# NoahVl/Explaining-In-Style-Reproducibility-Study

Hardware: AMD Instinct MI355X
Metric: StylEx G+D+enc train-step images/sec @256px (higher is better)
Workload: dtype bf16; 1 GPU; FFHQ-shaped 256x256 StylEx, batch 32/GPU, GAE=2 (noise+encoder micro-steps), GP every 4th step, ResNet-18 classifier; image_size=256, batch_per_gpu=32, start_step=0, gradient_accumulate_every=2, global_batch=32, parallelism=dp1

## Files before the change

explaining-in-style-reproducibility-study_amd/csrc/conv_gather.hip:

```cpp
#include <hip/hip_runtime.h>
#include <stdint.h>
#include <stdlib.h>

#include "conv_prims.h"
#include "stylex_internal.h"


namespace {


constexpr int GBM = 128, GBN = 128;
constexpr int RING = 4;

struct GatherParams {
    const unsigned short* x;
    const unsigned short* w;
    float* partial;
    unsigned short* y;
    int B, H, W, C, N, KH, pad, sign;
    int Hs, Ws, stride;
    int m_tiles;
    int M, stages, ksplit, stages_per_split;
};


constexpr int LROW = 128;
constexpr int LSTAGE = (GBM + GBN) * LROW;
constexpr int LPIECES = 4;

__device__ __forceinline__ void lds16(bf16x8& dst, int addr) {
    asm volatile("ds_read_b128 %0, %1" : "=v"(dst) : "v"(addr));
}

__global__ __launch_bounds__(512, 1) void conv_gather_line_kernel(GatherParams p) {
    extern __shared__ __attribute__((aligned(16))) char smem[];
    const int tid = threadIdx.x, lane = tid & 63;
    const int wave = __builtin_amdgcn_readfirstlane(tid >> 6);
    const int n_tiles = (p.N + GBN - 1) / GBN;
    const int n0 = (int)(blockIdx.x % n_tiles) * GBN;
    int mt = (int)(blockIdx.x / n_tiles);
    const bool phased = p.sign < 0 && p.stride == 2;
    int py = 0, px = 0;
    if (phased) {
        const int tpp = p.m_tiles >> 2;
        const int ph = mt / tpp;
        mt -= ph * tpp;
        py = ph >> 1;
        px = ph & 1;
    }
    const int m0 = mt * GBM;
    const int rows = phased ? p.B * p.Hs * p.Ws : p.M;
    const int cpt = p.C >> 6;
    const int ks = blockIdx.y;
    const int s_begin = ks * p.stages_per_split;
    const int s_end = min(s_begin + p.stages_per_split, phased ? (1 + py) * (1 + px) * cpt : p.stages);
    const int nst = max(s_end - s_begin, 0);
    const int T = p.KH * p.KH, K = T * p.C;

    const bool stage_w = wave >= 4;
    const int rbase = (wave & 3) * 32 + (lane >> 3);
    const int Hs = __builtin_amdgcn_readfirstlane(p.Hs), Ws = __builtin_amdgcn_readfirstlane(p.Ws);
    const int C = __builtin_amdgcn_readfirstlane(p.C), KH = __builtin_amdgcn_readfirstlane(p.KH);
    const int pad = __builtin_amdgcn_readfirstlane(p.pad), sgn = __builtin_amdgcn_readfirstlane(p.sign);
    const int strd = __builtin_amdgcn_readfirstlane(p.stride);
    const int gw = phased ? Ws : p.W;
    const int hw = phased ? Hs * Ws : p.H * p.W;
    const __amdgpu_buffer_rsrc_t rx = __builtin_amdgcn_make_buffer_rsrc(const_cast<unsigned short*>(p.x), 0, 0x7ffffff0, 0x00020000);
// ... 77 lines not shown
#pragma unroll
        for (int e = 0; e < 16; ++e) acc[j][e] = 0.f;

    for (int s = 0; s < 3 && s < nst; ++s) issue_stage(s);
    for (int s = 0; s < nst; ++s) {
        if (s + 2 < nst) asm volatile("s_waitcnt vmcnt(%0)" ::"n"(2 * LPIECES) : "memory");
        else if (s + 1 < nst) asm volatile("s_waitcnt vmcnt(%0)" ::"n"(LPIECES) : "memory");
        else asm volatile("s_waitcnt vmcnt(0)" ::: "memory");
        asm volatile("s_waitcnt lgkmcnt(0)" ::: "memory");
        __builtin_amdgcn_s_barrier();
        asm volatile("" ::: "memory");
        if (s + 3 < nst) issue_stage((s + 3) % RING);
        const int base = (s % RING) * LSTAGE;
        bf16x8 av[2], bv[2][2];
        lds16(av[0], base + a_off + (s0 << 4));
        lds16(bv[0][0], base + b_off + (s0 << 4));
        lds16(bv[0][1], base + b_off + 32 * LROW + (s0 << 4));
#pragma unroll
        for (int g = 0; g < 4; ++g) {
            if (g < 3) {
                const int so = ((2 * (g + 1)) ^ s0) << 4;
                lds16(av[(g + 1) & 1], base + a_off + so);
                lds16(bv[(g + 1) & 1][0], base + b_off + so);
                lds16(bv[(g + 1) & 1][1], base + b_off + 32 * LROW + so);
                asm volatile("s_waitcnt lgkmcnt(3)" : "+v"(av[g & 1]), "+v"(bv[g & 1][0]), "+v"(bv[g & 1][1]));
            } else {
                asm volatile("s_waitcnt lgkmcnt(0)" : "+v"(av[g & 1]), "+v"(bv[g & 1][0]), "+v"(bv[g & 1][1]));
            }
#pragma unroll
            for (int j = 0; j < 2; ++j) acc[j] = __builtin_amdgcn_mfma_f32_32x32x16_bf16(av[g & 1], bv[g & 1][j], acc[j], 0, 0, 0);
        }
    }

    float* out = p.partial + (long)ks * p.M * p.N;
#pragma unroll
    for (int j = 0; j < 2; ++j) {
        const int n = n0 + wn * 64 + j * 32 + li;
#pragma unroll
        for (int r = 0; r < 16; ++r) {
            int mm = m0 + wm * 32 + (r & 3) + 8 * (r >> 2) + 4 * lk;
            const bool ok = mm < rows && n < p.N;
            if (phased && ok) {
                const int bb = mm / hw, qq = mm - bb * hw;
                const int qh = qq / p.Ws, qw = qq - qh * p.Ws;
                mm = (bb * p.H + 2 * qh + py) * p.W + 2 * qw + px;
            }
            if (ok && p.y) p.y[(long)mm * p.N + n] = act_bf16_1(acc[j][r]);
            else if (ok) out[(long)mm * p.N + n] = acc[j][r];
        }
    }
}

}

static bool gather_applicable(const ConvKParams& p) {
    const char* env = getenv("STYLEX_CONV_GATHER");
    if (env && env[0] == '0') return false;
    if (env && env[0] == 's' && p.stride != 1) return false;
    if (!p.act_bf16 || p.a_scale || p.s2d_c) return false;
    if (p.KH != p.KW || !((p.KH == 3 && p.pad == 1) || (p.KH == 1 && p.pad == 0))) return false;
    if (p.stride == 1) {
        if (p.Hi != p.Ho || p.Wi != p.Wo || p.phase_major) return false;
    } else {
        if (p.stride != 2 || p.KH != 3) return false;
        if (p.transposed ? (p.Ho != 2 * p.Hi || p.Wo != 2 * p.Wi) : (p.Hi != 2 * p.Ho || p.Wi != 2 * p.Wo)) return false;
    }
    if ((p.transposed && p.stride == 2 ? p.Hi * p.Wi : p.Ho * p.Wo) > 64) return false;
    if (p.Ck % 64 != 0 || p.N % 8 != 0 || p.N < 64) return false;
    if ((reinterpret_cast<uintptr_t>(p.a) & 15) || (reinterpret_cast<uintptr_t>(p.w) & 15)) return false;
    return true;
}

static int gather_m_tiles(const ConvKParams& p) {
    if (p.transposed && p.stride == 2) return 4 * ((p.B * p.Hi * p.Wi + GBM - 1) / GBM);
    return (p.M + GBM - 1) / GBM;
}

static int gather_stages(const ConvKParams& p) {
    return (p.transposed && p.stride == 2 ? 4 : p.KH * p.KW) * (p.Ck / 64);
}

static void gather_plan(const ConvKParams& p, int* ksplit, int* per) {
    const int stages = gather_stages(p);
    const long tiles = (long)gather_m_tiles(p) * ((p.N + GBN - 1) / GBN);
    int ks = (int)((256 + tiles - 1) / tiles);
    if (ks > stages / 4) ks = stages / 4;
    if (ks < 1) ks = 1;
    int pp = (stages + ks - 1) / ks;
    *per = pp;
    *ksplit = (stages + pp - 1) / pp;
}

int64_t stylex_gather_workspace_bytes(const ConvKParams& p) {
    if (!gather_applicable(p)) return 0;
    int ks, per;
    gather_plan(p, &ks, &per);
    return (int64_t)ks * p.M * p.N * (int64_t)sizeof(float);
}

int stylex_launch_gather(ConvKParams& p, void* workspace, int64_t workspace_bytes, hipStream_t s) {
    if (!gather_applicable(p) || !workspace) return STYLEX_NOT_APPLICABLE;
    int ks, per;
    gather_plan(p, &ks, &per);
    if (workspace_bytes < (int64_t)ks * p.M * p.N * (int64_t)sizeof(float)) return STYLEX_NOT_APPLICABLE;
    if (reinterpret_cast<uintptr_t>(workspace) & 15) return STYLEX_NOT_APPLICABLE;
    if (stylex_dynamic_lds_once<conv_gather_line_kernel>(RING * LSTAGE) != hipSuccess) {
        (void)hipGetLastError();
        return STYLEX_NOT_APPLICABLE;
    }
    GatherParams g;
    g.x = reinterpret_cast<const unsigned short*>(p.a);
    g.w = reinterpret_cast<const unsigned short*>(p.w);
    g.partial = (float*)workspace;
    const bool direct = ks == 1 && p.flags == 0 && !p.out_scale && !p.bias;
    g.y = direct ? reinterpret_cast<unsigned short*>(p.y) : nullptr;
    g.B = p.B;
    g.H = p.Ho;
    g.W = p.Wo;
    g.C = p.Ck;
    g.N = p.N;
    g.KH = p.KH;
    g.pad = p.pad;
    g.sign = p.transposed ? -1 : 1;
    g.Hs = p.Hi;
    g.Ws = p.Wi;
    g.stride = p.stride;
    g.m_tiles = gather_m_tiles(p);
    g.M = p.M;
    g.stages = gather_stages(p);
    g.ksplit = ks;
    g.stages_per_split = per;
    const long tiles = (long)g.m_tiles * ((p.N + GBN - 1) / GBN);
    stylex_note_kernel("conv_gather_line_kernel");
    hipLaunchKernelGGL(conv_gather_line_kernel, dim3((unsigned)tiles, (unsigned)ks), dim3(512), RING * LSTAGE, s, g);
    p.ksplit = direct ? 0 : ks;
    p.kt_per_split = per;
    p.partial = (float*)workspace;
    return (int)hipGetLastError();
}
```

explaining-in-style-reproducibility-study_amd/csrc/conv_igemm.hip:

```cpp
#include <hip/hip_runtime.h>
#include <stdint.h>

#include "conv_prims.h"
#include "stylex_internal.h"


namespace {

constexpr int BK = 32;


struct RowPix {
    int b, oh, ow;
    bool valid;
};

__device__ __forceinline__ RowPix decode_row(const ConvKParams& p, int m) {
    RowPix r;
    r.valid = m < p.M;
    int mm = r.valid ? m : 0;
    if (p.phase_major) {
        int hh = p.Ho >> 1, wh = p.Wo >> 1;
        int per = p.B * hh * wh;
        int ph = mm / per;
// ... 739 lines not shown
        const unsigned mb = (unsigned)((pairs + 7) / 8);
        hipLaunchKernelGGL((wgrad_reduce_small_kernel<8, 32>), dim3(mb + extra), dim3(256), 0, s, partial, dw, N, C, T, splits,
                           (int)mb, bias_part, db, wo.scale, wo.accumulate);
    } else if (T <= 9 && splits >= 16 && pairs <= 16384) {
        const unsigned mb = (unsigned)((pairs + 31) / 32);
        hipLaunchKernelGGL((wgrad_reduce_small_kernel<32, 8>), dim3(mb + extra), dim3(256), 0, s, partial, dw, N, C, T, splits,
                           (int)mb, bias_part, db, wo.scale, wo.accumulate);
    } else {
        const unsigned mb = (unsigned)((pairs + 255) / 256);
        hipLaunchKernelGGL(wgrad_reduce_kernel, dim3(mb + extra), dim3(256), 0, s, partial, dw, N, C, T, splits, (int)mb,
                           bias_part, db, wo.scale, wo.accumulate);
    }
}

template <typename OUT>
__device__ __forceinline__ OUT cvt_out(float v);
template <>
__device__ __forceinline__ float cvt_out<float>(float v) { return v; }
template <>
__device__ __forceinline__ unsigned short cvt_out<unsigned short>(float v) { return act_bf16_1(v); }

template <typename OUT>
__global__ void pack_weight_kernel(const float* __restrict__ w, OUT* __restrict__ wf, OUT* __restrict__ wb, int N,
                                   int C, int T) {
    long total = (long)N * C * T;
    for (long i = blockIdx.x * (long)blockDim.x + threadIdx.x; i < total; i += (long)gridDim.x * blockDim.x) {
        int t = (int)(i % T);
        int c = (int)((i / T) % C);
        int n = (int)(i / ((long)T * C));
        OUT v = cvt_out<OUT>(w[i]);
        if (wf) wf[((long)n * T + t) * C + c] = v;
        if (wb) wb[((long)c * T + t) * N + n] = v;
    }
}

__device__ __forceinline__ float splitk_finish(const ConvKParams& p, float v, long o, int n, int b, int oh, int ow) {
    if (p.flags & STYLEX_EPI_OSCALE) v *= p.out_scale[(long)b * p.N + n];
    if (p.flags & STYLEX_EPI_BIAS) v += p.bias[n];
    if (p.flags & STYLEX_EPI_NOISE)
        v += ((p.flags & STYLEX_EPI_NOISE_NAT) ? p.noise[((long)b * p.noise_stride + oh) * p.noise_stride + ow]
                                               : p.noise[((long)b * p.noise_stride + ow) * p.noise_stride + oh]) * p.noise_w[n] + p.noise_b[n];
    if (p.flags & STYLEX_EPI_RESIDUAL) v = (v + act_ld1(p.residual, o, p.act_bf16)) * p.res_scale;
    if (p.flags & STYLEX_EPI_GATE) v = act_ld1(p.residual, o, p.act_bf16) > 0.f ? v : p.res_scale * v;
    if (p.flags & (STYLEX_EPI_LRELU | STYLEX_EPI_RELU)) v = v > 0.f ? v : ((p.flags & STYLEX_EPI_RELU) ? 0.f : 0.2f * v);
    return v;
}

template <bool VEC>
__global__ void splitk_epilogue_kernel(ConvKParams p) {
    const long total = (long)p.M * p.N;
    if (VEC) {
        const int tot = (int)total, N = p.N, hw = p.Ho * p.Wo;
        const bool need_pix = p.flags & (STYLEX_EPI_OSCALE | STYLEX_EPI_NOISE);
        for (int o = (blockIdx.x * blockDim.x + threadIdx.x) * 4; o < tot; o += gridDim.x * blockDim.x * 4) {
            float4 v = make_float4(0.f, 0.f, 0.f, 0.f);
            for (int s = 0; s < p.ksplit; ++s) {
                const float4 t = *reinterpret_cast<const float4*>(p.partial + (long)s * total + o);
                v.x += t.x; v.y += t.y; v.z += t.z; v.w += t.w;
            }
            const int pix = o / N, n = o - pix * N;
            int b = 0, oh = 0, ow = 0;
            if (need_pix) {
                b = pix / hw;
                const int q = pix - b * hw;
                oh = q / p.Wo;
                ow = q - oh * p.Wo;
            }
            float r[4] = {v.x, v.y, v.z, v.w};
#pragma unroll
            for (int e = 0; e < 4; ++e) r[e] = splitk_finish(p, r[e], (long)o + e, n + e, b, oh, ow);
            if (p.act_bf16) {
                uint2 h;
                h.x = act_pack2(r[0], r[1]);
                h.y = act_pack2(r[2], r[3]);
                *reinterpret_cast<uint2*>(reinterpret_cast<unsigned short*>(p.y) + o) = h;
            } else {
                *reinterpret_cast<float4*>(reinterpret_cast<float*>(p.y) + o) = make_float4(r[0], r[1], r[2], r[3]);
            }
// ... 309 lines not shown
```

explaining-in-style-reproducibility-study_amd/csrc/stylex_capi.hip:

```cpp
#include <hip/hip_runtime.h>
#include <stdint.h>
#include <stdarg.h>
#include <stdio.h>
#include <string.h>

#include <array>
#include <map>
#include <mutex>
#include <string>
#include <vector>

#include "stylex_internal.h"

namespace {

typedef std::array<int64_t, 9> LayerKey;
struct TimedLaunch {
    hipEvent_t start, stop;
    int cls;
    double flops;
    double bytes;
    LayerKey key;
    char kernel[112];
};
// ... 205 lines not shown

static void fwd_params(ConvKParams& p, const int64_t* sh) {
    fill_common(p, sh);
    p.Hi = (int)sh[1];
    p.Wi = (int)sh[2];
    p.Ck = (int)sh[3];
    p.N = (int)sh[4];
    p.Ho = (int)sh[9];
    p.Wo = (int)sh[10];
    p.M = p.B * p.Ho * p.Wo;
}

static void bwd_data_params(ConvKParams& p, const int64_t* sh) {
    fill_common(p, sh);
    p.Hi = (int)sh[9];
    p.Wi = (int)sh[10];
    p.Ck = (int)sh[4];
    p.N = (int)sh[3];
    p.Ho = (int)sh[1];
    p.Wo = (int)sh[2];
    p.M = p.B * p.Ho * p.Wo;
}

int64_t stylex_conv2d_workspace_bytes(const int64_t* sh, int which, int precision) {
    if (!conv_shape_ok(sh) || (which != 0 && which != 1)) return STYLEX_EINVAL;
    ConvKParams p;
    if (which == 0) fwd_params(p, sh);
    else {
        bwd_data_params(p, sh);
        p.transposed = 1;
    }
    p.act_bf16 = precision == STYLEX_BF16_ACT;
    return stylex_igemm_workspace_bytes(p, precision);
}

int stylex_conv_mask_supported(const int64_t* sh, int which, int flags, int precision) {
    if (!conv_shape_ok(sh) || precision != STYLEX_BF16_ACT || (which != 0 && which != 1)) return 0;
    static const uintptr_t fake = 4096;
    ConvKParams p;
    if (which == 0) {
        if (!(flags & STYLEX_EPI_MASK_OUT) || !(flags & STYLEX_EPI_LRELU)) return 0;
        fwd_params(p, sh);
        if (p.N % 8 != 0) return 0;
        p.mask = (unsigned char*)fake;
    } else {
        if (!(flags & STYLEX_EPI_GATE_MASK) || (flags & ~(STYLEX_EPI_GATE_MASK))) return 0;
        bwd_data_params(p, sh);
        if (p.KH != 3 || p.stride != 1 || p.pad != 1) return 0;
        p.flip_taps = 1;
        p.gate_mask = (const unsigned char*)fake;
    }
    p.a = (const float*)fake;
    p.w = (const void*)fake;
    p.y = (float*)fake;
    p.bias = (const float*)fake;
    p.flags = flags;
    p.act_bf16 = 1;
    p.dry = 1;
    if (which == 0 && stylex_launch_rgb(p, nullptr) == 0) return 1;
    return stylex_launch_halo(p, nullptr) == 0 ? 1 : 0;
}

int stylex_conv2d_fwd(const void* x, const void* w_fwd, void* y, const int64_t* sh, int flags,
                      const stylex_conv_epilogue* epi, int precision, void* workspace, int64_t workspace_bytes,
                      void* stream) {
    if (!x || !w_fwd || !y || !conv_shape_ok(sh)) return STYLEX_EINVAL;
// ... 263 lines not shown
```

explaining-in-style-reproducibility-study_amd/csrc/stylex_internal.h:

```cpp
#pragma once
#include <hip/hip_runtime.h>
#include <stdint.h>

#include "../../include/stylex_hip.h"
#include "act_io.h"

struct ConvKParams {
    const float* a;
    const float* a_scale;
    const void* w;
    const float* a2;
    const float* a2_scale;
    float* y;
    const float* bias;
    const float* out_scale;
    const float* noise;
    const float* noise_w;
    const float* noise_b;
    const float* residual;
    float res_scale;
    int noise_stride;
    int B, Hi, Wi, Ck, N, KH, KW, Ho, Wo, stride, pad;
    int transposed;
    int phase_major;
    int act_bf16;
    int s2d_c;
    int flip_taps;
    int M;
    int flags;
    long split_len;
    int ksplit;
    int kt_per_split;
    float* partial;
    unsigned char* mask;
    const unsigned char* gate_mask;
    int dry;
    float* bias_partial;
    const void* x2;
    const void* w2;
    int c2;
    float wg_scale;
    int wg_accumulate;
};

int stylex_launch_igemm(ConvKParams p, int precision, void* workspace, int64_t workspace_bytes, hipStream_t s);
int64_t stylex_igemm_workspace_bytes(const ConvKParams& p, int precision);
void stylex_wgrad_plan(const ConvKParams& p, int* tn, int* tc, int* splits, long* split_len);
int stylex_launch_wgrad(ConvKParams p, float* partial, float* dw_oihw, int precision, hipStream_t s, float* db = nullptr,
                        int* db_done = nullptr);
int stylex_launch_pack(const float* w, void* wf, void* wb, int N, int C, int T, int dtype, hipStream_t s);

#define STYLEX_NOT_APPLICABLE (-100)

int stylex_cu_count();

template <auto Kernel>
hipError_t stylex_dynamic_lds_once(int bytes) {
    static const hipError_t e =
        hipFuncSetAttribute(reinterpret_cast<const void*>(Kernel), hipFuncAttributeMaxDynamicSharedMemorySize, bytes);
    return e;
}

void stylex_note_kernel(const char* fmt, ...);
#define STYLEX_TIMING_INPUT 3
class StylexTimedCall {
  public:
    StylexTimedCall(int cls, double bytes, hipStream_t s);
    ~StylexTimedCall();
    StylexTimedCall(const StylexTimedCall&) = delete;
    StylexTimedCall& operator=(const StylexTimedCall&) = delete;

  private:
    void* impl_;
};

#ifdef __HIPCC__
__device__ __forceinline__ unsigned stylex_sign_bits8(uint4 v) {
    const unsigned w[4] = {v.x, v.y, v.z, v.w};
    unsigned m = 0;
#pragma unroll
    for (int d = 0; d < 4; ++d) {
        m |= (__uint_as_float(w[d] << 16) > 0.f ? 1u : 0u) << (2 * d);
        m |= (__uint_as_float(w[d] & 0xffff0000u) > 0.f ? 1u : 0u) << (2 * d + 1);
    }
    return m;
}
#endif
int stylex_launch_halo(const ConvKParams& p, hipStream_t s);

int stylex_launch_halo_dma(const ConvKParams& p, hipStream_t s);

int stylex_launch_rgb(const ConvKParams& p, hipStream_t s);

int stylex_launch_pipe(const ConvKParams& p, hipStream_t s);
int stylex_launch_line64(const ConvKParams& p, hipStream_t s);

int stylex_launch_s2d_dgrad(const ConvKParams& p, hipStream_t s);
int stylex_launch_s2d_fwd(const ConvKParams& p, hipStream_t s);

int stylex_launch_gather(ConvKParams& p, void* workspace, int64_t workspace_bytes, hipStream_t s);
int64_t stylex_gather_workspace_bytes(const ConvKParams& p);

bool stylex_wgrad_pipe_applicable(const ConvKParams& p);
void stylex_wgrad_pipe_plan(const ConvKParams& p, int* slices, int* tiles_per_split, int* blocks);
int stylex_launch_wgrad_pipe(ConvKParams p, float* partial, hipStream_t s, int* slices_out, int* bias_done = nullptr);
int stylex_launch_wgrad_s2d_folded(ConvKParams p, float* partial, float* dw_oihw, hipStream_t s);

bool stylex_wgrad_tr_applicable(const ConvKParams& p);
void stylex_wgrad_tr_plan(const ConvKParams& p, int* mode, int* splits, long* split_len);
int stylex_launch_wgrad_tr(ConvKParams p, float* partial, hipStream_t s, int* splits_out);

__host__ __device__ inline unsigned stylex_s2d_tap_mask(int s) {
    const int sy = s >> 1, sx = s & 1;
    unsigned m = 0;
    for (int kh = 0; kh < 2; ++kh)
        for (int kw = 0; kw < 2; ++kw)
            if ((kh == 1 || sy == 1) && (kw == 1 || sx == 1)) m |= 1u << (kh * 3 + kw);
    return m;
}
int stylex_launch_pack_s2d(const float* w, void* wf, void* wb, int N, int C, hipStream_t s);
int stylex_launch_fold_s2d(const float* dw2, float* dw, int N, int C, hipStream_t s);
```

explaining-in-style-reproducibility-study_amd/stylex/hip_backend.py:

```python
import os as _os

if _os.environ.get("STYLEX_MIOPEN_ALLOW_BWD_GTC", "0") != "1":
    _os.environ.setdefault("MIOPEN_DEBUG_CONV_IMPLICIT_GEMM_ASM_BWD_GTC_XDLOPS_NHWC", "0")

import atexit
import ctypes
import os
import weakref

import torch

import operand_cache
from operand_cache import mark_updated, packs, stamp as _gen, vectors

_HERE = os.path.dirname(os.path.abspath(__file__))
LIB_PATH = os.path.join(os.path.dirname(_HERE), "libstylex_hip.so")

F32, BF16, BF16_ACT = 0, 1, 2
EPI_BIAS, EPI_LRELU, EPI_OSCALE, EPI_NOISE, EPI_RESIDUAL, EPI_RELU, EPI_GATE, EPI_NOISE_NAT = 1, 2, 4, 8, 16, 32, 64, 128
EPI_MASK_OUT, EPI_GATE_MASK = 256, 512

_c_f = ctypes.c_void_p
_i64p = ctypes.POINTER(ctypes.c_int64)


class ConvEpilogue(ctypes.Structure):
    _fields_ = [
        ("in_scale", ctypes.c_void_p),
        ("bias", ctypes.c_void_p),
        ("out_scale", ctypes.c_void_p),
        ("noise", ctypes.c_void_p),
        ("noise_stride", ctypes.c_int64),
        ("noise_w", ctypes.c_void_p),
        ("noise_b", ctypes.c_void_p),
        ("residual", ctypes.c_void_p),
        ("res_scale", ctypes.c_float),
        ("s2d_c", ctypes.c_int32),
        ("mask", ctypes.c_void_p),
    ]


SIGNATURES = {
    "stylex_init": (ctypes.c_int, [ctypes.c_int]),
    "stylex_version": (ctypes.c_char_p, []),
    "stylex_pack_weight": (ctypes.c_int, [_c_f, _c_f, _c_f, _i64p, ctypes.c_int, ctypes.c_void_p]),
    "stylex_conv2d_workspace_bytes": (ctypes.c_int64, [_i64p, ctypes.c_int, ctypes.c_int]),
    "stylex_conv2d_fwd": (ctypes.c_int, [_c_f, _c_f, _c_f, _i64p, ctypes.c_int, ctypes.POINTER(ConvEpilogue),
                                         ctypes.c_int, ctypes.c_void_p, ctypes.c_int64, ctypes.c_void_p]),
    "stylex_conv2d_bwd_data": (ctypes.c_int, [_c_f, _c_f, _c_f, _i64p, ctypes.c_int, ctypes.POINTER(ConvEpilogue),
                                              ctypes.c_int, ctypes.c_void_p, ctypes.c_int64, ctypes.c_void_p]),
    "stylex_conv2d_bwd_weight_workspace_bytes": (ctypes.c_int64, [_i64p]),
    "stylex_conv2d_bwd_weight": (ctypes.c_int, [_c_f, _c_f, _c_f, ctypes.c_void_p, ctypes.c_int64, _i64p, _c_f, _c_f,
                                                ctypes.c_int, ctypes.c_int, ctypes.c_void_p]),
    "stylex_conv2d_bwd_weight_bias": (ctypes.c_int, [_c_f, _c_f, _c_f, _c_f, ctypes.POINTER(ctypes.c_int), ctypes.c_void_p,
                                                     ctypes.c_int64, _i64p, _c_f, _c_f, ctypes.c_int, ctypes.c_int,
                                                     ctypes.c_void_p]),
    "stylex_conv2d_bwd_weight_ex": (ctypes.c_int, [_c_f, _c_f, _c_f, _c_f, ctypes.POINTER(ctypes.c_int), ctypes.c_void_p,
                                                   ctypes.c_int64, _i64p, _c_f, _c_f, ctypes.c_int, ctypes.c_float, ctypes.c_int,
                                                   ctypes.c_int, ctypes.c_void_p]),
    "stylex_blur3x3_s2d_fwd": (ctypes.c_int, [_c_f, _c_f, _i64p, ctypes.c_int, ctypes.c_void_p]),
    "stylex_blur3x3_s2d_bwd": (ctypes.c_int, [_c_f, _c_f, _i64p, ctypes.c_int, ctypes.c_void_p]),
    "stylex_blur3x3_reflect_bwd_gate": (ctypes.c_int, [_c_f, _c_f, ctypes.c_float, _c_f, _i64p, ctypes.c_int, ctypes.c_void_p]),
    "stylex_blur3x3_s2d_bwd_gate": (ctypes.c_int, [_c_f, _c_f, ctypes.c_float, _c_f, _i64p, ctypes.c_int, ctypes.c_void_p]),
    "stylex_blur3x3_s2d_bwd_gate_mask": (ctypes.c_int, [_c_f, _c_f, ctypes.c_float, _c_f, _i64p, ctypes.c_int, ctypes.c_void_p]),
    "stylex_conv_mask_supported": (ctypes.c_int, [_i64p, ctypes.c_int, ctypes.c_int, ctypes.c_int]),
    "stylex_add_at_even": (ctypes.c_int, [_c_f, _c_f, _i64p, ctypes.c_int, ctypes.c_void_p]),
    "stylex_subsample2_fwd": (ctypes.c_int, [_c_f, _c_f, _i64p, ctypes.c_int, ctypes.c_void_p]),
    "stylex_subsample2_bwd": (ctypes.c_int, [_c_f, _c_f, _i64p, ctypes.c_int, ctypes.c_void_p]),
    "stylex_pack_weight_s2d": (ctypes.c_int, [_c_f, _c_f, _c_f, _i64p, ctypes.c_void_p]),
    "stylex_fold_weight_grad_s2d": (ctypes.c_int, [_c_f, _c_f, _i64p, ctypes.c_void_p]),
    "stylex_conv2d_bwd_weight_s2d_supported": (ctypes.c_int, [_i64p, ctypes.c_int, ctypes.c_int]),
    "stylex_conv2d_bwd_weight_s2d": (ctypes.c_int, [ctypes.c_void_p, ctypes.c_void_p, _c_f, ctypes.c_void_p, ctypes.c_int64, _i64p,
                                                    ctypes.c_int, ctypes.c_float, ctypes.c_int, ctypes.c_int, ctypes.c_void_p]),
    "stylex_upsample2x_bilinear_fwd": (ctypes.c_int, [_c_f, _c_f, _i64p, ctypes.c_int, ctypes.c_void_p]),
    "stylex_upsample2x_bilinear_bwd": (ctypes.c_int, [_c_f, _c_f, _i64p, ctypes.c_int, ctypes.c_void_p]),
    "stylex_rgb_up_blur_add_fwd": (ctypes.c_int, [_c_f, _c_f, _c_f, _i64p, ctypes.c_int, ctypes.c_void_p]),
    "stylex_rgb_up_blur_add_bwd": (ctypes.c_int, [_c_f, _c_f, _i64p, ctypes.c_int, ctypes.c_void_p]),
    "stylex_blur3x3_reflect_fwd": (ctypes.c_int, [_c_f, _c_f, _i64p, ctypes.c_int, ctypes.c_void_p]),
    "stylex_blur3x3_reflect_bwd": (ctypes.c_int, [_c_f, _c_f, _i64p, ctypes.c_int, ctypes.c_void_p]),
# ... 96 lines not shown
    "stylex_linattn_chunks": (ctypes.c_int, [_i64p]),
    "stylex_linattn_fwd": (ctypes.c_int, [_c_f, _c_f, _c_f, _i64p, _c_f, _c_f, _c_f, _c_f, _c_f, _i64p, ctypes.c_int,
                                          ctypes.c_void_p]),
    "stylex_linattn_bwd": (ctypes.c_int, [_c_f, _c_f, _c_f, _i64p] + [_c_f] * 8 + [_i64p, ctypes.c_int, ctypes.c_void_p]),
    "stylex_chan_norm_fwd": (ctypes.c_int, [_c_f] * 6 + [_i64p, ctypes.c_float, ctypes.c_int, ctypes.c_void_p]),
    "stylex_chan_norm_bwd_blocks": (ctypes.c_int, [_i64p]),
    "stylex_chan_norm_bwd": (ctypes.c_int, [_c_f] * 8 + [_i64p, ctypes.c_float, ctypes.c_int, ctypes.c_void_p]),
    "stylex_dwconv3x3_fwd": (ctypes.c_int, [_c_f, _c_f, _c_f, _i64p, ctypes.c_int, ctypes.c_void_p]),
    "stylex_dwconv3x3_wgrad_blocks": (ctypes.c_int, [_i64p]),
    "stylex_dwconv3x3_bwd_weight": (ctypes.c_int, [_c_f, _c_f, _c_f, _c_f, _i64p, ctypes.c_int, ctypes.c_void_p]),
    "stylex_initial_block_supported": (ctypes.c_int, [_i64p]),
    "stylex_initial_block_fwd": (ctypes.c_int, [_c_f, _c_f, _c_f, _i64p, ctypes.c_int, ctypes.c_int, ctypes.c_void_p]),
    "stylex_initial_block_bwd_data": (ctypes.c_int, [_c_f, _c_f, _c_f, _i64p, ctypes.c_int, ctypes.c_int, ctypes.c_void_p]),
    "stylex_initial_block_bwd_weight": (ctypes.c_int, [_c_f, _c_f, _c_f, _i64p, ctypes.c_int, ctypes.c_void_p]),
    "stylex_resample_rows_u8": (ctypes.c_int, [ctypes.c_void_p, _c_f, ctypes.c_int64, ctypes.c_int64, ctypes.c_int64, _c_f,
                                               ctypes.c_int64, _c_f, ctypes.c_int64, ctypes.c_void_p]),
    "stylex_resample_cols_u8": (ctypes.c_int, [ctypes.c_void_p, _c_f, ctypes.c_int64, ctypes.c_int64, ctypes.c_int64, _c_f,
                                               ctypes.c_int64, _c_f, ctypes.c_int64, _c_f, _c_f, ctypes.c_int64,
                                               ctypes.c_void_p]),
    "stylex_crop_lut_u8": (ctypes.c_int, [ctypes.c_void_p, _c_f, ctypes.c_int64, ctypes.c_int64, ctypes.c_int64, _c_f,
                                          ctypes.c_int64, _c_f, _c_f, ctypes.c_int64, ctypes.c_void_p]),
    "stylex_timing_report": (ctypes.c_int, [ctypes.c_int, _i64p, ctypes.POINTER(ctypes.c_double),
                                            ctypes.POINTER(ctypes.c_double), ctypes.POINTER(ctypes.c_double)]),
}

_lib = None
_inited_devices = set()


class StylexHipError(RuntimeError):
    pass


OPTIONAL_SYMBOLS = frozenset(["stylex_modconv_bwd_prep_nat"])
_MISSING_OPTIONAL = set()


def has_symbol(name):
    load_library()
    return name not in _MISSING_OPTIONAL


def load_library(path=None):
    global _lib
    if _lib is not None:
        return _lib
    path = path or os.environ.get("STYLEX_HIP_LIB", LIB_PATH)
    if not os.path.isfile(path):
        raise StylexHipError("libstylex_hip.so not found at %s — run `python __graft_entry__.py build` "
                             "(there is no CPU fallback for the product path)" % path)
    lib = ctypes.CDLL(path)
    _MISSING_OPTIONAL.clear()
    for name, (res, args) in SIGNATURES.items():
        if name in OPTIONAL_SYMBOLS and path != LIB_PATH and not hasattr(lib, name):
            _MISSING_OPTIONAL.add(name)
            continue
        fn = getattr(lib, name)
        fn.restype = res
        fn.argtypes = args
    if os.environ.get("STYLEX_SYNC_TRACE", "0") == "1":
        lib = _SyncTraced(lib)
    _lib = lib
    return lib


class _SyncTraced:

# ... 430 lines not shown
        ws = _empty(max(nbytes // 4, 1), dtype=torch.float32, device=x2.device)
        dw = accumulate_into if accumulate_into is not None else _empty((n, c, 3, 3), dtype=torch.float32, device=x2.device)
        assert tuple(dw.shape) == (n, c, 3, 3) and (isinstance(dw, RawGrad) or (dw.dtype == torch.float32 and dw.is_contiguous()))
        _check(lib.stylex_conv2d_bwd_weight_s2d(_ptr(x2), _ptr(dy), _ptr(dw), _ptr(ws), nbytes, shp, c, float(out_scale),
                                                int(accumulate_into is not None), precision, _stream()),
               "stylex_conv2d_bwd_weight_s2d")
        return None if isinstance(dw, RawGrad) else dw
    dw = fold_weight_grad_s2d(conv2d_bwd_weight(x2, dy, ws2, 1, 1, precision, s2d_c=c), (n, c, 3, 3))
    if out_scale != 1.0:
        dw.mul_(out_scale)
    if isinstance(accumulate_into, RawGrad):
        return dw
    if accumulate_into is not None:
        return accumulate_into.add_(dw)
    return dw


def fold_weight_grad_s2d(dw2, w_shape):
    lib = _ensure_device(dw2)
    n, c = w_shape[0], w_shape[1]
    dw = _empty(tuple(w_shape), dtype=torch.float32, device=dw2.device)
    _check(lib.stylex_fold_weight_grad_s2d(_ptr(dw2.contiguous()), _ptr(dw), _shape(n, c, 3, 3), _stream()),
           "stylex_fold_weight_grad_s2d")
    return dw


def _split_workspace(lib, shp, which, precision, like):
    nbytes = lib.stylex_conv2d_workspace_bytes(shp, which, precision)
    if nbytes <= 0:
        return None, 0
    return _empty(nbytes // 4, dtype=torch.float32, device=like.device), nbytes


_MASK_OK = {}


def conv_mask_supported(sh, which, flags, precision):
    key = (tuple(sh), which, flags, precision)
    hit = _MASK_OK.get(key)
    if hit is None:
        hit = _MASK_OK[key] = bool(load_library().stylex_conv_mask_supported(_shape(*sh), which, flags, precision))
    return hit


_S2D_RES_OK = {}


def s2d_res_supported(xb_shape, n, s2d_c, res_c):
    key = (tuple(xb_shape), n, s2d_c, res_c)
    hit = _S2D_RES_OK.get(key)
    if hit is None:
        sh = conv_shape(xb_shape, (n, xb_shape[1], 3, 3), 1, 1)
        hit = _S2D_RES_OK[key] = bool(load_library().stylex_conv2d_s2d_res_supported(_shape(*sh), s2d_c, res_c))
    return hit


def conv2d_s2d_res_fwd(xb, wf2, xs, w_res_mat, bias, n, s2d_c, scale):
    lib = _ensure_device(xb)
    assert is_cl(xb) and is_cl(xs) and xb.dtype == torch.bfloat16 and xs.dtype == torch.bfloat16
    assert xs.shape[0] == xb.shape[0] and xs.shape[2:] == xb.shape[2:] and w_res_mat.shape == (n, xs.shape[1])
    sh = conv_shape(xb.shape, (n, xb.shape[1], 3, 3), 1, 1)
    y = empty_cl((sh[0], n, sh[9], sh[10]), xb, torch.bfloat16)
    bias = _f32(bias)
    _check(lib.stylex_conv2d_s2d_res_fwd(_ptr(xb), _ptr(wf2), _ptr(xs), _ptr(w_res_mat), _ptr(bias), _ptr(y), _shape(*sh),
                                         int(s2d_c), int(xs.shape[1]), float(scale), _stream()), "stylex_conv2d_s2d_res_fwd")
    return y
# ... 1214 lines not shown
```

include/stylex_hip.h:

```cpp
#ifndef STYLEX_HIP_H
#define STYLEX_HIP_H

#include <stdint.h>

#ifdef __cplusplus
extern "C" {
#endif

#define STYLEX_F32 0
#define STYLEX_BF16 1
#define STYLEX_BF16_ACT 2

#define STYLEX_EINVAL (-1)
#define STYLEX_EWORKSPACE (-2)

#define STYLEX_CONV_NSHAPE 11

#define STYLEX_EPI_BIAS 1
#define STYLEX_EPI_LRELU 2
#define STYLEX_EPI_OSCALE 4
#define STYLEX_EPI_NOISE 8
#define STYLEX_EPI_RESIDUAL 16
#define STYLEX_EPI_RELU 32
#define STYLEX_EPI_NOISE_NAT 128
#define STYLEX_EPI_MASK_OUT 256
#define STYLEX_EPI_GATE_MASK 512
#define STYLEX_EPI_GATE 64

int stylex_init(int device);
const char* stylex_version(void);

int stylex_pack_weight(const float* w_oihw, void* w_fwd, void* w_bwd, const int64_t* shape, int precision,
                       void* stream);

typedef struct {
    const float* in_scale;
    const float* bias;
    const float* out_scale;
    const float* noise;
    int64_t noise_stride;
    const float* noise_w;
    const float* noise_b;
    const void* residual;
    float res_scale;
    int32_t s2d_c;
    void* mask;
} stylex_conv_epilogue;

int stylex_conv_mask_supported(const int64_t* shape, int which, int flags, int precision);

int64_t stylex_conv2d_workspace_bytes(const int64_t* shape, int which, int precision);

int stylex_conv2d_fwd(const void* x, const void* w_fwd, void* y, const int64_t* shape, int flags,
                      const stylex_conv_epilogue* epi, int precision, void* workspace, int64_t workspace_bytes,
                      void* stream);

int stylex_conv2d_s2d_res_supported(const int64_t* shape, int64_t s2d_c, int64_t res_c);
int stylex_conv2d_s2d_res_fwd(const void* x_s2d, const void* w_fwd_s2d, const void* x_res, const void* w_res, const float* bias,
                              void* y, const int64_t* shape, int64_t s2d_c, int64_t res_c, float scale, void* stream);

int stylex_conv2d_bwd_data(const void* dy, const void* w_bwd, void* dx, const int64_t* shape, int flags,
                           const stylex_conv_epilogue* epi, int precision, void* workspace, int64_t workspace_bytes,
                           void* stream);

int64_t stylex_conv2d_bwd_weight_workspace_bytes(const int64_t* shape);
int stylex_conv2d_bwd_weight(const void* x, const void* dy, float* dw, void* workspace, int64_t workspace_bytes,
                             const int64_t* shape, const float* x_scale, const float* dy_scale, int s2d_c,
                             int precision, void* stream);
int stylex_conv2d_bwd_weight_bias(const void* x, const void* dy, float* dw, float* db, int* db_written, void* workspace,
                                  int64_t workspace_bytes, const int64_t* shape, const float* x_scale,
                                  const float* dy_scale, int s2d_c, int precision, void* stream);
int stylex_conv2d_bwd_weight_ex(const void* x, const void* dy, float* dw, float* db, int* db_written, void* workspace,
                                int64_t workspace_bytes, const int64_t* shape, const float* x_scale, const float* dy_scale,
                                int s2d_c, float out_scale, int accumulate, int precision, void* stream);

int stylex_upsample2x_bilinear_fwd(const void* x, void* y, const int64_t* shape, int act_dtype, void* stream);
int stylex_upsample2x_bilinear_bwd(const void* dy, void* dx, const int64_t* shape, int act_dtype, void* stream);

int stylex_blur3x3_reflect_fwd(const void* x, void* y, const int64_t* shape, int act_dtype, void* stream);
int stylex_blur3x3_reflect_bwd(const void* dy, void* dx, const int64_t* shape, int act_dtype, void* stream);

int stylex_rgb_up_blur_add_fwd(const void* rgb, const void* prev, void* out, const int64_t* shape, int act_dtype,
                               void* stream);
int stylex_rgb_up_blur_add_bwd(const void* dy, void* dx, const int64_t* shape, int act_dtype, void* stream);
// ... 204 lines not shown
```

Baseline: 1006 images/sec.

## Fuse split-K epilogue into gather conv kernel when no K-split is needed

When the gather conv plan uses a single K slice, the kernel now stages the accumulator tile through LDS and applies the full epilogue (output scale, bias, noise, residual, gate, activation) in-kernel, writing packed bf16 vectors directly. Previously this direct path was only taken when no epilogue flags were set, so other cases wrote fp32 partials to workspace and ran a separate finish pass. The fused path removes that extra kernel and the fp32 round trip, at the cost of an LDS transpose with extra barriers and more register pressure in the epilogue. It also adds an env override for the K-split count and a plan-query API exposed to Python.

```diff
diff --git a/explaining-in-style-reproducibility-study_amd/csrc/conv_gather.hip b/explaining-in-style-reproducibility-study_amd/csrc/conv_gather.hip
--- a/explaining-in-style-reproducibility-study_amd/csrc/conv_gather.hip
+++ b/explaining-in-style-reproducibility-study_amd/csrc/conv_gather.hip
@@ -1,6 +1,8 @@
 #include <hip/hip_runtime.h>
 #include <stdint.h>
 #include <stdlib.h>
+
+#include <type_traits>
 
 #include "conv_prims.h"
 #include "stylex_internal.h"
@@ -32,7 +34,12 @@
     asm volatile("ds_read_b128 %0, %1" : "=v"(dst) : "v"(addr));
 }
 
-__global__ __launch_bounds__(512, 1) void conv_gather_line_kernel(GatherParams p) {
+struct NoEpilogue {};
+template <bool FUSED>
+using EpilogueOf = std::conditional_t<FUSED, ConvKParams, NoEpilogue>;
+
+template <bool FUSED>
+__global__ __launch_bounds__(512, 1) void conv_gather_line_kernel(GatherParams p, EpilogueOf<FUSED> e) {
     extern __shared__ __attribute__((aligned(16))) char smem[];
     const int tid = threadIdx.x, lane = tid & 63;
     const int wave = __builtin_amdgcn_readfirstlane(tid >> 6);
@@ -176,21 +183,66 @@
         }
     }
 
-    float* out = p.partial + (long)ks * p.M * p.N;
-#pragma unroll
-    for (int j = 0; j < 2; ++j) {
-        const int n = n0 + wn * 64 + j * 32 + li;
-#pragma unroll
-        for (int r = 0; r < 16; ++r) {
-            int mm = m0 + wm * 32 + (r & 3) + 8 * (r >> 2) + 4 * lk;
-            const bool ok = mm < rows && n < p.N;
-            if (phased && ok) {
-                const int bb = mm / hw, qq = mm - bb * hw;
-                const int qh = qq / p.Ws, qw = qq - qh * p.Ws;
-                mm = (bb * p.H + 2 * qh + py) * p.W + 2 * qw + px;
-            }
-            if (ok && p.y) p.y[(long)mm * p.N + n] = act_bf16_1(acc[j][r]);
-            else if (ok) out[(long)mm * p.N + n] = acc[j][r];
+    if constexpr (!FUSED) {
+        float* out = p.partial + (long)ks * p.M * p.N;
+#pragma unroll
+        for (int j = 0; j < 2; ++j) {
+            const int n = n0 + wn * 64 + j * 32 + li;
+#pragma unroll
+            for (int r = 0; r < 16; ++r) {
+                int mm = m0 + wm * 32 + (r & 3) + 8 * (r >> 2) + 4 * lk;
+                const bool ok = mm < rows && n < p.N;
+                if (phased && ok) {
+                    const int bb = mm / hw, qq = mm - bb * hw;
+                    const int qh = qq / p.Ws, qw = qq - qh * p.Ws;
+                    mm = (bb * p.H + 2 * qh + py) * p.W + 2 * qw + px;
+                }
+                if (ok) out[(long)mm * p.N + n] = acc[j][r];
+            }
+        }
+    } else {
+        __syncthreads();
+        float* ot = reinterpret_cast<float*>(smem);
+#pragma unroll
+        for (int j = 0; j < 2; ++j) {
+            float* dst = ot + (wm * 32 + 4 * lk) * GBN + wn * 64 + ((j ^ lk) << 5) + li;
+#pragma unroll
+            for (int r = 0; r < 16; ++r) dst[((r & 3) + 8 * (r >> 2)) * GBN] = acc[j][r];
+        }
+        __syncthreads();
+        const bool need_pix = e.flags & (STYLEX_EPI_OSCALE | STYLEX_EPI_NOISE);
+#pragma unroll
+        for (int q = 0; q < (GBM * GBN / 8) / 512; ++q) {
+            const int u = tid + q * 512;
+            const int row = u >> 4, col = (u & 15) << 3;
+            const float* src = ot + row * GBN + (col ^ (((row >> 2) & 1) << 5));
+            const float4 l0 = *reinterpret_cast<const float4*>(src), l1 = *reinterpret_cast<const float4*>(src + 4);
+            float v[8] = {l0.x, l0.y, l0.z, l0.w, l1.x, l1.y, l1.z, l1.w};
+            int mm = m0 + row;
+            const int n = n0 + col;
+            if (mm >= rows || n >= p.N) continue;
+            int b = 0, oh = 0, ow = 0;
+            if (phased) {
+                b = mm / hw;
+                const int qq = mm - b * hw, qh = qq / p.Ws;
+                oh = 2 * qh + py;
+                ow = 2 * (qq - qh * p.Ws) + px;
+                mm = (b * p.H + oh) * p.W + ow;
+            } else if (need_pix) {
+                b = mm / hw;
+                const int qq = mm - b * hw;
+                oh = qq / p.W;
+                ow = qq - oh * p.W;
+            }
+            const long o = (long)mm * p.N + n;
+#pragma unroll
+            for (int c = 0; c < 8; ++c) v[c] = splitk_finish(e, v[c], o + c, n + c, b, oh, ow);
+            uint4 h;
+            h.x = act_pack2(v[0], v[1]);
+            h.y = act_pack2(v[2], v[3]);
+            h.z = act_pack2(v[4], v[5]);
+            h.w = act_pack2(v[6], v[7]);
+            *reinterpret_cast<uint4*>(p.y + o) = h;
         }
     }
 }
@@ -229,10 +281,17 @@
     const long tiles = (long)gather_m_tiles(p) * ((p.N + GBN - 1) / GBN);
     int ks = (int)((256 + tiles - 1) / tiles);
     if (ks > stages / 4) ks = stages / 4;
+    const char* env = getenv("STYLEX_GATHER_KSPLIT");
+    if (env && atoi(env) > 0) ks = atoi(env) < stages ? atoi(env) : stages;
     if (ks < 1) ks = 1;
     int pp = (stages + ks - 1) / ks;
     *per = pp;
     *ksplit = (stages + pp - 1) / pp;
+}
+
+static bool gather_fused_epilogue() {
+    const char* env = getenv("STYLEX_GATHER_FUSED_EPI");
+    return !(env && env[0] == '0');
 }
 
 int64_t stylex_gather_workspace_bytes(const ConvKParams& p) {
@@ -240,6 +299,16 @@
     int ks, per;
     gather_plan(p, &ks, &per);
     return (int64_t)ks * p.M * p.N * (int64_t)sizeof(float);
+}
+
+int stylex_gather_plan_query(const ConvKParams& p, int32_t* plan) {
+    if (!gather_applicable(p)) return 0;
+    int ks, per;
+    gather_plan(p, &ks, &per);
+    plan[0] = ks;
+    plan[1] = per;
+    plan[2] = ks == 1 && gather_fused_epilogue() ? 1 : 0;
+    return 1;
 }
 
 int stylex_launch_gather(ConvKParams& p, void* workspace, int64_t workspace_bytes, hipStream_t s) {
@@ -248,7 +317,8 @@
     gather_plan(p, &ks, &per);
     if (workspace_bytes < (int64_t)ks * p.M * p.N * (int64_t)sizeof(float)) return STYLEX_NOT_APPLICABLE;
     if (reinterpret_cast<uintptr_t>(workspace) & 15) return STYLEX_NOT_APPLICABLE;
-    if (stylex_dynamic_lds_once<conv_gather_line_kernel>(RING * LSTAGE) != hipSuccess) {
+    if (stylex_dynamic_lds_once<conv_gather_line_kernel<false>>(RING * LSTAGE) != hipSuccess ||
+        stylex_dynamic_lds_once<conv_gather_line_kernel<true>>(RING * LSTAGE) != hipSuccess) {
         (void)hipGetLastError();
         return STYLEX_NOT_APPLICABLE;
     }
@@ -256,7 +326,7 @@
     g.x = reinterpret_cast<const unsigned short*>(p.a);
     g.w = reinterpret_cast<const unsigned short*>(p.w);
     g.partial = (float*)workspace;
-    const bool direct = ks == 1 && p.flags == 0 && !p.out_scale && !p.bias;
+    const bool direct = ks == 1 && gather_fused_epilogue() && !(reinterpret_cast<uintptr_t>(p.y) & 15);
     g.y = direct ? reinterpret_cast<unsigned short*>(p.y) : nullptr;
     g.B = p.B;
     g.H = p.Ho;
@@ -276,7 +346,10 @@
     g.stages_per_split = per;
     const long tiles = (long)g.m_tiles * ((p.N + GBN - 1) / GBN);
     stylex_note_kernel("conv_gather_line_kernel");
-    hipLaunchKernelGGL(conv_gather_line_kernel, dim3((unsigned)tiles, (unsigned)ks), dim3(512), RING * LSTAGE, s, g);
+    if (direct)
+        hipLaunchKernelGGL(conv_gather_line_kernel<true>, dim3((unsigned)tiles, 1u), dim3(512), RING * LSTAGE, s, g, p);
+    else
+        hipLaunchKernelGGL(conv_gather_line_kernel<false>, dim3((unsigned)tiles, (unsigned)ks), dim3(512), RING * LSTAGE, s, g, NoEpilogue{});
     p.ksplit = direct ? 0 : ks;
     p.kt_per_split = per;
     p.partial = (float*)workspace;
diff --git a/explaining-in-style-reproducibility-study_amd/csrc/conv_igemm.hip b/explaining-in-style-reproducibility-study_amd/csrc/conv_igemm.hip
--- a/explaining-in-style-reproducibility-study_amd/csrc/conv_igemm.hip
+++ b/explaining-in-style-reproducibility-study_amd/csrc/conv_igemm.hip
@@ -795,18 +795,6 @@
         if (wf) wf[((long)n * T + t) * C + c] = v;
         if (wb) wb[((long)c * T + t) * N + n] = v;
     }
-}
-
-__device__ __forceinline__ float splitk_finish(const ConvKParams& p, float v, long o, int n, int b, int oh, int ow) {
-    if (p.flags & STYLEX_EPI_OSCALE) v *= p.out_scale[(long)b * p.N + n];
-    if (p.flags & STYLEX_EPI_BIAS) v += p.bias[n];
-    if (p.flags & STYLEX_EPI_NOISE)
-        v += ((p.flags & STYLEX_EPI_NOISE_NAT) ? p.noise[((long)b * p.noise_stride + oh) * p.noise_stride + ow]
-                                               : p.noise[((long)b * p.noise_stride + ow) * p.noise_stride + oh]) * p.noise_w[n] + p.noise_b[n];
-    if (p.flags & STYLEX_EPI_RESIDUAL) v = (v + act_ld1(p.residual, o, p.act_bf16)) * p.res_scale;
-    if (p.flags & STYLEX_EPI_GATE) v = act_ld1(p.residual, o, p.act_bf16) > 0.f ? v : p.res_scale * v;
-    if (p.flags & (STYLEX_EPI_LRELU | STYLEX_EPI_RELU)) v = v > 0.f ? v : ((p.flags & STYLEX_EPI_RELU) ? 0.f : 0.2f * v);
-    return v;
 }
 
 template <bool VEC>
diff --git a/explaining-in-style-reproducibility-study_amd/csrc/stylex_capi.hip b/explaining-in-style-reproducibility-study_amd/csrc/stylex_capi.hip
--- a/explaining-in-style-reproducibility-study_amd/csrc/stylex_capi.hip
+++ b/explaining-in-style-reproducibility-study_amd/csrc/stylex_capi.hip
@@ -261,6 +261,19 @@
     }
     p.act_bf16 = precision == STYLEX_BF16_ACT;
     return stylex_igemm_workspace_bytes(p, precision);
+}
+
+int stylex_conv2d_gather_plan(const int64_t* sh, int which, int precision, int32_t* plan) {
+    if (!plan || !conv_shape_ok(sh) || (which != 0 && which != 1)) return STYLEX_EINVAL;
+    if (precision != STYLEX_BF16_ACT) return 0;
+    ConvKParams p;
+    if (which == 0) fwd_params(p, sh);
+    else {
+        bwd_data_params(p, sh);
+        p.transposed = 1;
+    }
+    p.act_bf16 = 1;
+    return stylex_gather_plan_query(p, plan);
 }
 
 int stylex_conv_mask_supported(const int64_t* sh, int which, int flags, int precision) {
diff --git a/explaining-in-style-reproducibility-study_amd/csrc/stylex_internal.h b/explaining-in-style-reproducibility-study_amd/csrc/stylex_internal.h
--- a/explaining-in-style-reproducibility-study_amd/csrc/stylex_internal.h
+++ b/explaining-in-style-reproducibility-study_amd/csrc/stylex_internal.h
@@ -42,6 +42,33 @@
     float wg_scale;
     int wg_accumulate;
 };
+
+#ifdef __HIPCC__
+__device__ __forceinline__ float splitk_chain(int flags, float res_scale, float v, float os, float bi, float nz, float nw, float nb,
+                                              float rs) {
+#pragma clang fp contract(off)
+    if (flags & STYLEX_EPI_OSCALE) v *= os;
+    if (flags & STYLEX_EPI_BIAS) v += bi;
+    if (flags & STYLEX_EPI_NOISE) v += __builtin_fmaf(nz, nw, nb);
+    if (flags & STYLEX_EPI_RESIDUAL) v = (v + rs) * res_scale;
+    if (flags & STYLEX_EPI_GATE) v = rs > 0.f ? v : res_scale * v;
+    if (flags & (STYLEX_EPI_LRELU | STYLEX_EPI_RELU)) v = v > 0.f ? v : ((flags & STYLEX_EPI_RELU) ? 0.f : 0.2f * v);
+    return v;
+}
+__device__ __forceinline__ float splitk_finish(const ConvKParams& p, float v, long o, int n, int b, int oh, int ow) {
+    float os = 0.f, bi = 0.f, nz = 0.f, nw = 0.f, nb = 0.f, rs = 0.f;
+    if (p.flags & STYLEX_EPI_OSCALE) os = p.out_scale[(long)b * p.N + n];
+    if (p.flags & STYLEX_EPI_BIAS) bi = p.bias[n];
+    if (p.flags & STYLEX_EPI_NOISE) {
+        nz = (p.flags & STYLEX_EPI_NOISE_NAT) ? p.noise[((long)b * p.noise_stride + oh) * p.noise_stride + ow]
+                                              : p.noise[((long)b * p.noise_stride + ow) * p.noise_stride + oh];
+        nw = p.noise_w[n];
+        nb = p.noise_b[n];
+    }
+    if (p.flags & (STYLEX_EPI_RESIDUAL | STYLEX_EPI_GATE)) rs = act_ld1(p.residual, o, p.act_bf16);
+    return splitk_chain(p.flags, p.res_scale, v, os, bi, nz, nw, nb, rs);
+}
+#endif
 
 int stylex_launch_igemm(ConvKParams p, int precision, void* workspace, int64_t workspace_bytes, hipStream_t s);
 int64_t stylex_igemm_workspace_bytes(const ConvKParams& p, int precision);
@@ -100,6 +127,7 @@
 
 int stylex_launch_gather(ConvKParams& p, void* workspace, int64_t workspace_bytes, hipStream_t s);
 int64_t stylex_gather_workspace_bytes(const ConvKParams& p);
+int stylex_gather_plan_query(const ConvKParams& p, int32_t* plan);
 
 bool stylex_wgrad_pipe_applicable(const ConvKParams& p);
 void stylex_wgrad_pipe_plan(const ConvKParams& p, int* slices, int* tiles_per_split, int* blocks);
diff --git a/explaining-in-style-reproducibility-study_amd/stylex/hip_backend.py b/explaining-in-style-reproducibility-study_amd/stylex/hip_backend.py
--- a/explaining-in-style-reproducibility-study_amd/stylex/hip_backend.py
+++ b/explaining-in-style-reproducibility-study_amd/stylex/hip_backend.py
@@ -45,6 +45,7 @@
     "stylex_version": (ctypes.c_char_p, []),
     "stylex_pack_weight": (ctypes.c_int, [_c_f, _c_f, _c_f, _i64p, ctypes.c_int, ctypes.c_void_p]),
     "stylex_conv2d_workspace_bytes": (ctypes.c_int64, [_i64p, ctypes.c_int, ctypes.c_int]),
+    "stylex_conv2d_gather_plan": (ctypes.c_int, [_i64p, ctypes.c_int, ctypes.c_int, ctypes.POINTER(ctypes.c_int32)]),
     "stylex_conv2d_fwd": (ctypes.c_int, [_c_f, _c_f, _c_f, _i64p, ctypes.c_int, ctypes.POINTER(ConvEpilogue),
                                          ctypes.c_int, ctypes.c_void_p, ctypes.c_int64, ctypes.c_void_p]),
     "stylex_conv2d_bwd_data": (ctypes.c_int, [_c_f, _c_f, _c_f, _i64p, ctypes.c_int, ctypes.POINTER(ConvEpilogue),
@@ -207,7 +208,7 @@
     pass
 
 
-OPTIONAL_SYMBOLS = frozenset(["stylex_modconv_bwd_prep_nat"])
+OPTIONAL_SYMBOLS = frozenset(["stylex_modconv_bwd_prep_nat", "stylex_conv2d_gather_plan"])
 _MISSING_OPTIONAL = set()
 
 
@@ -704,6 +705,16 @@
     return _empty(nbytes // 4, dtype=torch.float32, device=like.device), nbytes
 
 
+def gather_plan(sh, which, precision):
+    lib = load_library()
+    if not has_symbol("stylex_conv2d_gather_plan"):
+        return None
+    plan = (ctypes.c_int32 * 3)()
+    rc = lib.stylex_conv2d_gather_plan(_shape(*sh), which, precision, plan)
+    _check(min(rc, 0), "stylex_conv2d_gather_plan")
+    return dict(slices=plan[0], stages=plan[1], fused=bool(plan[2])) if rc == 1 else None
+
+
 _MASK_OK = {}
 
 
diff --git a/include/stylex_hip.h b/include/stylex_hip.h
--- a/include/stylex_hip.h
+++ b/include/stylex_hip.h
@@ -50,6 +50,8 @@
 int stylex_conv_mask_supported(const int64_t* shape, int which, int flags, int precision);
 
 int64_t stylex_conv2d_workspace_bytes(const int64_t* shape, int which, int precision);
+
+int stylex_conv2d_gather_plan(const int64_t* shape, int which, int precision, int32_t* plan);
 
 int stylex_conv2d_fwd(const void* x, const void* w_fwd, void* y, const int64_t* shape, int flags,
                       const stylex_conv_epilogue* epi, int precision, void* workspace, int64_t workspace_bytes,
```

Result: no change. 1006 images/sec (-0.0%).
